# UncertainLab/Enlsip.jl

Measured on NVIDIA B200. Metric: batched CNLS solves/s (n=6,m=128), higher is better.
Workload: dtype f64

## Files before the change

### enlsip.jl_b200/csrc/enl_base.h

```cpp
#pragma once
#include <math.h>
#include <stdint.h>
#include <type_traits>

#if defined(__CUDACC__)
#define ENL_FN __device__
#define ENL_INL __device__ __forceinline__
#define ENL_NOINL __device__ __noinline__
#else
#define ENL_FN
#define ENL_INL inline
#define ENL_NOINL
#endif

namespace enl {

#if defined(__CUDA_ARCH__)
ENL_INL double mul_rn(double a, double b) { return __dmul_rn(a, b); }
ENL_INL double add_rn(double a, double b) { return __dadd_rn(a, b); }
ENL_INL double sub_rn(double a, double b) { return __dsub_rn(a, b); }
ENL_INL double fma_rn(double a, double b, double c) { return fma(a, b, c); }
ENL_INL double div_rn(double a, double b) { return __ddiv_rn(a, b); }
ENL_INL double sqrt_rn(double a) { return __dsqrt_rn(a); }
#else
ENL_INL double mul_rn(double a, double b) { return a * b; }
ENL_INL double add_rn(double a, double b) { return a + b; }
ENL_INL double sub_rn(double a, double b) { return a - b; }
ENL_INL double fma_rn(double a, double b, double c) { return __builtin_fma(a, b, c); }
ENL_INL double div_rn(double a, double b) { return a / b; }
ENL_INL double sqrt_rn(double a) { return sqrt(a); }
#endif

ENL_INL double div_z(double a, double b) { return (a == 0.0) ? a : div_rn(a, b); }

ENL_INL double pow2i(int k) {
    long long b = (long long)(k + 1023) << 52;
#if defined(__CUDA_ARCH__)
    return __longlong_as_double(b);
#else
    double d;
    __builtin_memcpy(&d, &b, 8);
    return d;
#endif
}

#if defined(ENL_COMPACT_CODE) && defined(__CUDA_ARCH__)
#define ENL_DET_EXP_ATTR ENL_NOINL
#else
#define ENL_DET_EXP_ATTR ENL_INL
#endif
ENL_DET_EXP_ATTR double det_exp(double x) {
    const double LOG2E = 1.44269504088896338700e+00;
    const double LN2_HI = 6.93147180369123816490e-01;
    const double LN2_LO = 1.90821492927058770002e-10;
    double xc = fmin(fmax(x, -800.0), 710.0);
    double kd = rint(mul_rn(xc, LOG2E));
    int k = (int)kd;
    double r = fma_rn(-kd, LN2_HI, xc);
    r = fma_rn(-kd, LN2_LO, r);
    double acc = 1.0 / 6227020800.0;
    acc = fma_rn(acc, r, 1.0 / 479001600.0);
    acc = fma_rn(acc, r, 1.0 / 39916800.0);
    acc = fma_rn(acc, r, 1.0 / 3628800.0);
    acc = fma_rn(acc, r, 1.0 / 362880.0);
    acc = fma_rn(acc, r, 1.0 / 40320.0);
    acc = fma_rn(acc, r, 1.0 / 5040.0);
    acc = fma_rn(acc, r, 1.0 / 720.0);
    acc = fma_rn(acc, r, 1.0 / 120.0);
    acc = fma_rn(acc, r, 1.0 / 24.0);
    acc = fma_rn(acc, r, 1.0 / 6.0);
    acc = fma_rn(acc, r, 0.5);
    acc = fma_rn(acc, r, 1.0);
    acc = fma_rn(acc, r, 1.0);
    int k1 = k >> 1;
    int k2 = k - k1;
    double res = mul_rn(mul_rn(acc, pow2i(k1)), pow2i(k2));
    if (x < -745.2) res = 0.0;
    if (x > 709.782712893384) res = INFINITY;
    return (x != x) ? x : res;
}

ENL_INL double det_tanh(double z) {
    double e = det_exp(mul_rn(2.0, z));
    return sub_rn(1.0, div_rn(2.0, add_rn(e, 1.0)));
}

#if defined(__CUDACC__)
template <int G_>
struct DevGroup {
    static constexpr int G = G_;
    unsigned mask;
    int lane;
    __device__ DevGroup() {
        int wl = threadIdx.x & 31;
        lane = wl & (G - 1);
        mask = (G == 32) ? 0xffffffffu : (((1u << G) - 1u) << (wl & ~(G - 1)));
    }
    __device__ __forceinline__ void sync() const {
        if (G > 1) __syncwarp(mask);
    }
    __device__ __forceinline__ double sum(double v) const {
#pragma unroll
        for (int o = G / 2; o > 0; o >>= 1) v += __shfl_xor_sync(mask, v, o, G);
        return v;
    }
    __device__ __forceinline__ double maxv(double v) const {
#pragma unroll
        for (int o = G / 2; o > 0; o >>= 1) v = fmax(v, __shfl_xor_sync(mask, v, o, G));
        return v;
    }
};
#endif

struct HostGroup {
    static constexpr int G = 1;
    int lane = 0;
    void sync() const {}
    double sum(double v) const { return v; }
    double maxv(double v) const { return v; }
};

#if defined(__CUDACC__)
extern __shared__ __align__(16) double enl_smem[];
using vref = int;
ENL_INL vref make_vref(double* p) { return (int)(p - enl_smem); }
ENL_INL vref make_vref(int* p) { return (int)(p - reinterpret_cast<int*>(enl_smem)); }
ENL_INL double& vderef_d(vref o) { return enl_smem[o]; }
ENL_INL int& vderef_i(vref o) { return reinterpret_cast<int*>(enl_smem)[o]; }
#else
using vref = void*;
ENL_INL vref make_vref(double* p) { return p; }
ENL_INL vref make_vref(int* p) { return p; }
#endif

template <int S>
struct SV {
#if defined(__CUDACC__)
    int p;
    ENL_INL double& operator[](int i) const { return enl_smem[p + i * S]; }
#else
    double* p;
    ENL_INL double& operator[](int i) const { return p[i * S]; }
#endif
    ENL_INL SV off(int k) const { return SV{p + k * S}; }
};
template <int S>
struct SI {
#if defined(__CUDACC__)
    int p;
    ENL_INL int& operator[](int i) const { return reinterpret_cast<int*>(enl_smem)[p + i * S]; }
#else
    int* p;
    ENL_INL int& operator[](int i) const { return p[i * S]; }
#endif
};

template <int G, int MS, int NT>
struct DM {
#if defined(__CUDACC__)
    int grp;
    ENL_INL static int lane() { return (int)(threadIdx.x & (G - 1)); }
    ENL_INL static int row_of(int s) { return s * G + lane(); }
    ENL_INL double& at(int s, int c) const { return enl_smem[grp + lane() + (c * MS + s) * NT]; }
    ENL_INL double& row(int r, int c) const { return enl_smem[grp + (c * MS + r / G) * NT + (r % G)]; }
#else
    double* grp;
    ENL_INL static int row_of(int s) { return s * G; }
    ENL_INL double& at(int s, int c) const { return grp[(c * MS + s) * NT]; }
    ENL_INL double& row(int r, int c) const { return grp[(c * MS + r / G) * NT + (r % G)]; }
#endif
    ENL_INL DM cols(int c0) const { return DM{grp + c0 * MS * NT}; }
};

ENL_INL double sq(double v) { return v * v; }
ENL_INL int imin(int a, int b) { return a < b ? a : b; }
ENL_INL int imax(int a, int b) { return a > b ? a : b; }
ENL_INL double sign_of(double a, double b) { return b >= 0.0 ? fabs(a) : -fabs(a); }

ENL_INL double lapy2(double x, double y) {
    double xa = fabs(x), ya = fabs(y);
    double w = fmax(xa, ya), z = fmin(xa, ya);
    if (z == 0.0 || w > 1.7e308) return w;
    return w * sqrt(1.0 + (z / w) * (z / w));
}

constexpr double EPS = 2.220446049250313e-16;
constexpr double SQRT_EPS = 1.4901161193847656e-08;
constexpr double TOL3Z = 1.0536712127723509e-08;

constexpr int EXIT_WOULD_THROW = -99;
constexpr int EXIT_WOULD_HANG = -98;
constexpr int EXIT_CAPACITY = -97;

}
```

### enlsip.jl_b200/csrc/enl_linalg.h

```cpp
#pragma once
#include "enl_base.h"

namespace enl {

#if defined(ENL_HOST_BUILD)
typedef void (*host_dgeqp3_fn)(const int*, const int*, double*, const int*, int*, double*, double*, const int*, int*);
inline host_dgeqp3_fn& host_dgeqp3() { static host_dgeqp3_fn fn = nullptr; return fn; }
inline void host_lapack_qrcp(double* a, int ld, int rows, int cols, double* tau, int* jpvt) {
    static thread_local double work[8192];
    for (int j = 0; j < cols; ++j) jpvt[j] = 0;
    int info = 0;
    const int lwork = 8192;
    host_dgeqp3()(&rows, &cols, a, &ld, jpvt, tau, work, &lwork, &info);
    for (int j = 0; j < cols; ++j) jpvt[j] -= 1;
}
#endif

template <class V>
ENL_NOINL double nrm2_small(V a, int n) {
    double s = 0.0;
#pragma unroll 1
    for (int i = 0; i < n; ++i) s += a[i] * a[i];
    return sqrt(s);
}

template <class V, class VI>
ENL_NOINL void qrcp_small(V a, int ld, int rows, int cols, V tau, VI jpvt, V vn1, V vn2) {
#if defined(ENL_HOST_BUILD)
    if (host_dgeqp3() && rows > 0 && cols > 0) { host_lapack_qrcp(&a[0], ld, rows, cols, &tau[0], &jpvt[0]); return; }
#endif
#pragma unroll 1
    for (int j = 0; j < cols; ++j) {
        jpvt[j] = j;
        double nj = nrm2_small(a.off(j * ld), rows);
        vn1[j] = nj;
        vn2[j] = nj;
    }
    int k = imin(rows, cols);
#pragma unroll 1
    for (int i = 0; i < k; ++i) {
        int pvt = i;
        double best = vn1[i];
#pragma unroll 1
        for (int j = i + 1; j < cols; ++j)
            if (vn1[j] > best) { best = vn1[j]; pvt = j; }
        if (pvt != i) {
#pragma unroll 1
            for (int r = 0; r < rows; ++r) {
                double tmp = a[pvt * ld + r];
                a[pvt * ld + r] = a[i * ld + r];
                a[i * ld + r] = tmp;
            }
            int it = jpvt[pvt]; jpvt[pvt] = jpvt[i]; jpvt[i] = it;
            vn1[pvt] = vn1[i];
            vn2[pvt] = vn2[i];
        }
        double tau_i = 0.0;
        if (i < rows - 1) {
            double alpha = a[i * ld + i];
            double xn = nrm2_small(a.off(i * ld + i + 1), rows - i - 1);
            if (xn != 0.0) {
                double beta = -sign_of(lapy2(alpha, xn), alpha);
                tau_i = (beta - alpha) / beta;
                double sc = 1.0 / (alpha - beta);
#pragma unroll 1
                for (int r = i + 1; r < rows; ++r) a[i * ld + r] *= sc;
                a[i * ld + i] = beta;
            }
        }
        tau[i] = tau_i;
        if (i < cols - 1 && tau_i != 0.0) {
#pragma unroll 1
            for (int c = i + 1; c < cols; ++c) {
                double wv = a[c * ld + i];
#pragma unroll 1
                for (int r = i + 1; r < rows; ++r) wv += a[i * ld + r] * a[c * ld + r];
                wv *= tau_i;
                a[c * ld + i] -= wv;
#pragma unroll 1
                for (int r = i + 1; r < rows; ++r) a[c * ld + r] -= wv * a[i * ld + r];
            }
        }
#pragma unroll 1
        for (int j = i + 1; j < cols; ++j) {
            double v1 = vn1[j];
            if (v1 != 0.0) {
                double tq = fabs(a[j * ld + i]) / v1;
                double temp = fmax(1.0 - tq * tq, 0.0);
                double rq = v1 / vn2[j];
                double temp2 = temp * (rq * rq);
                if (temp2 <= TOL3Z) {
                    if (i < rows - 1) {
                        double nj = nrm2_small(a.off(j * ld + i + 1), rows - i - 1);
                        vn1[j] = nj;
                        vn2[j] = nj;
                    } else {
                        vn1[j] = 0.0;
                        vn2[j] = 0.0;
                    }
                } else {
                    vn1[j] = v1 * sqrt(temp);
                }
            }
        }
    }
}

template <class V>
ENL_NOINL void apply_qt_small(V a, int ld, int rows, int k, V tau, V v) {
#pragma unroll 1
    for (int i = 0; i < k; ++i) {
        double ti = tau[i];
        if (ti == 0.0) continue;
        double wv = v[i];
#pragma unroll 1
        for (int r = i + 1; r < rows; ++r) wv += a[i * ld + r] * v[r];
        wv *= ti;
        v[i] -= wv;
#pragma unroll 1
        for (int r = i + 1; r < rows; ++r) v[r] -= wv * a[i * ld + r];
    }
}

template <class V>
ENL_NOINL void apply_q_small(V a, int ld, int rows, int k, V tau, V v) {
#pragma unroll 1
    for (int i = k - 1; i >= 0; --i) {
        double ti = tau[i];
        if (ti == 0.0) continue;
        double wv = v[i];
#pragma unroll 1
        for (int r = i + 1; r < rows; ++r) wv += a[i * ld + r] * v[r];
        wv *= ti;
        v[i] -= wv;
#pragma unroll 1
        for (int r = i + 1; r < rows; ++r) v[r] -= wv * a[i * ld + r];
    }
}

template <class V, class V2>
ENL_NOINL bool solve_upper_small(V R, int ld, int k, V2 x) {
#pragma unroll 1
    for (int i = k - 1; i >= 0; --i) {
        double s = x[i];
#pragma unroll 1
        for (int j = i + 1; j < k; ++j) s -= R[j * ld + i] * x[j];
        double d = R[i * ld + i];
        if (d == 0.0) return false;
        x[i] = s / d;
    }
    return true;
}

template <class V, class V2>
ENL_NOINL bool solve_upperT_small(V R, int ld, int k, V2 x) {
#pragma unroll 1
    for (int i = 0; i < k; ++i) {
        double s = x[i];
#pragma unroll 1
        for (int j = 0; j < i; ++j) s -= R[i * ld + j] * x[j];
        double d = R[i * ld + i];
        if (d == 0.0) return false;
        x[i] = s / d;
    }
    return true;
}

template <class V>
ENL_NOINL int pseudo_rank(V R, int ld, int len, double eps_rank) {
    if (len <= 0 || fabs(R[0]) < eps_rank) return 0;
    double tol = fabs(R[0]) * sqrt((double)len) * eps_rank;
    int r = 1;
#pragma unroll 1
    while (r < len && fabs(R[(r - 1) * ld + (r - 1)]) > tol) ++r;
    return r - ((r == len && fabs(R[(r - 1) * ld + (r - 1)]) > tol) ? 0 : 1);
}

template <class Grp, int G, int MS, int NT>
struct Dist {
    Grp g;

    ENL_NOINL double colsq(DM<G, MS, NT> a, int c, int r0) const {
        double s = 0.0;
#pragma unroll
        for (int sl = 0; sl < MS; ++sl) {
            int row = sl * G + g.lane;
            double v = a.at(sl, c);
            if (row >= r0) s += v * v;
        }
        return g.sum(s);
    }

    template <class V>
    ENL_NOINL void mul_q_right(DM<G, MS, NT> J, int n, V fa, int ld, int k, V tau) const {
#pragma unroll 1
        for (int i = 0; i < k; ++i) {
            double ti = tau[i];
            if (ti == 0.0) continue;
#pragma unroll
            for (int sl = 0; sl < MS; ++sl) {
                double wv = J.at(sl, i);
#pragma unroll 1
                for (int c = i + 1; c < n; ++c) wv += J.at(sl, c) * fa[i * ld + c];
                wv *= ti;
                J.at(sl, i) -= wv;
#pragma unroll 1
                for (int c = i + 1; c < n; ++c) J.at(sl, c) -= wv * fa[i * ld + c];
            }
        }
    }

    template <class V, class VI>
    ENL_NOINL void qrcp(DM<G, MS, NT> a, int M, int ncols, V tau2, VI jpvt, V vn1, V vn2, V Rout, int ldr) const {
#if defined(ENL_HOST_BUILD)
        if (host_dgeqp3() && G == 1 && NT == 1 && M > 0 && ncols > 0) {
            host_lapack_qrcp(&a.at(0, 0), MS, M, ncols, &tau2[0], &jpvt[0]);
            const int kk = imin(M, ncols);
            for (int c = 0; c < ncols; ++c)
                for (int r = 0; r < kk; ++r) Rout[c * ldr + r] = (r <= c) ? a.row(r, c) : 0.0;
            return;
        }
#endif
#pragma unroll 1
        for (int j = 0; j < ncols; ++j) {
            jpvt[j] = j;
            double nj = sqrt(colsq(a, j, 0));
            vn1[j] = nj;
            vn2[j] = nj;
        }
        int k = imin(M, ncols);
#pragma unroll 1
        for (int i = 0; i < k; ++i) {
            int pvt = i;
            double best = vn1[i];
#pragma unroll 1
            for (int j = i + 1; j < ncols; ++j)
                if (vn1[j] > best) { best = vn1[j]; pvt = j; }
            if (pvt != i) {
#pragma unroll
                for (int sl = 0; sl < MS; ++sl) {
                    double tmp = a.at(sl, pvt);
                    a.at(sl, pvt) = a.at(sl, i);
                    a.at(sl, i) = tmp;
                }
                int it = jpvt[pvt]; jpvt[pvt] = jpvt[i]; jpvt[i] = it;
                vn1[pvt] = vn1[i];
                vn2[pvt] = vn2[i];
            }
            g.sync();
            double tau_i = 0.0;
            if (i < M - 1) {
                double alpha = a.row(i, i);
                double xn = sqrt(colsq(a, i, i + 1));
                if (xn != 0.0) {
                    double beta = -sign_of(lapy2(alpha, xn), alpha);
                    tau_i = (beta - alpha) / beta;
                    double sc = 1.0 / (alpha - beta);
                    g.sync();
#pragma unroll
                    for (int sl = 0; sl < MS; ++sl) {
                        int row = sl * G + g.lane;
                        if (row > i) a.at(sl, i) *= sc;
                        else if (row == i) a.at(sl, i) = beta;
                    }
                }
            }
            tau2[i] = tau_i;
            if (i < ncols - 1 && tau_i != 0.0) {
#pragma unroll 1
                for (int c = i + 1; c < ncols; ++c) {
                    double part = 0.0;
#pragma unroll
                    for (int sl = 0; sl < MS; ++sl) {
                        int row = sl * G + g.lane;
                        double vv = (row > i) ? a.at(sl, i) : ((row == i) ? 1.0 : 0.0);
                        part += vv * a.at(sl, c);
                    }
                    double wv = g.sum(part) * tau_i;
#pragma unroll
                    for (int sl = 0; sl < MS; ++sl) {
                        int row = sl * G + g.lane;
                        if (row > i) a.at(sl, c) -= wv * a.at(sl, i);
                        else if (row == i) a.at(sl, c) -= wv;
                    }
                }
            }
            g.sync();
#pragma unroll 1
            for (int j = i + 1; j < ncols; ++j) {
                double v1 = vn1[j];
                if (v1 != 0.0) {
                    double tq = fabs(a.row(i, j)) / v1;
                    double temp = fmax(1.0 - tq * tq, 0.0);
                    double rq = v1 / vn2[j];
                    double temp2 = temp * (rq * rq);
                    if (temp2 <= TOL3Z) {
                        if (i < M - 1) {
                            double nj = sqrt(colsq(a, j, i + 1));
                            vn1[j] = nj;
                            vn2[j] = nj;
                        } else {
                            vn1[j] = 0.0;
                            vn2[j] = 0.0;
                        }
                    } else {
                        vn1[j] = v1 * sqrt(temp);
                    }
                }
            }
        }
        g.sync();
#pragma unroll 1
        for (int c = 0; c < ncols; ++c)
#pragma unroll 1
            for (int r = 0; r < k; ++r) Rout[c * ldr + r] = (r <= c) ? a.row(r, c) : 0.0;
    }

    template <class V>
    ENL_NOINL void apply_qt(DM<G, MS, NT> a, int k, V tau2, DM<G, MS, NT> d) const {
#pragma unroll 1
        for (int i = 0; i < k; ++i) {
            double ti = tau2[i];
            if (ti == 0.0) continue;
            double part = 0.0;
#pragma unroll
            for (int sl = 0; sl < MS; ++sl) {
                int row = sl * G + g.lane;
                double vv = (row > i) ? a.at(sl, i) : ((row == i) ? 1.0 : 0.0);
                part += vv * d.at(sl, 0);
            }
            double wv = g.sum(part) * ti;
#pragma unroll
            for (int sl = 0; sl < MS; ++sl) {
                int row = sl * G + g.lane;
                if (row > i) d.at(sl, 0) -= wv * a.at(sl, i);
                else if (row == i) d.at(sl, 0) -= wv;
            }
        }
        g.sync();
    }

    template <class V>
    ENL_NOINL void apply_q_regs(DM<G, MS, NT> a, int k, V tau2, double* v) const {
#pragma unroll 1
        for (int i = k - 1; i >= 0; --i) {
            double ti = tau2[i];
            if (ti == 0.0) continue;
            double part = 0.0;
#pragma unroll
            for (int sl = 0; sl < MS; ++sl) {
                int row = sl * G + g.lane;
                double vv = (row > i) ? a.at(sl, i) : ((row == i) ? 1.0 : 0.0);
                part += vv * v[sl];
            }
            double wv = g.sum(part) * ti;
#pragma unroll
            for (int sl = 0; sl < MS; ++sl) {
                int row = sl * G + g.lane;
                double vv = (row > i) ? a.at(sl, i) : ((row == i) ? 1.0 : 0.0);
                v[sl] -= wv * vv;
            }
        }
    }

    ENL_NOINL double prefix_sq(DM<G, MS, NT> d, int len) const {
        double s = 0.0;
#pragma unroll
        for (int sl = 0; sl < MS; ++sl) {
            int row = sl * G + g.lane;
            double v = d.at(sl, 0);
            if (row < len) s += v * v;
        }
        return g.sum(s);
    }
};

}
```

### enlsip.jl_b200/csrc/enl_solver.h

```cpp
#pragma once
#include "enl_base.h"
#include "enl_linalg.h"
#include "enl_families.h"

namespace enl {

struct Options {
    int max_iter;
    int scaling;
    int jac_mode;
    int second_derivatives;
    double time_limit;
    double eps_abs;
    double eps_rel;
    double eps_x;
    double eps_c;
    double eps_rank;
};

constexpr int MAX_N = 32;
struct Bounds {
    int nlo, nup;
    int lo_idx[MAX_N], up_idx[MAX_N];
    double lo_val[MAX_N], up_val[MAX_N];
};

constexpr int TRACE_HDR = 16;

template <class Fam, int G, int NT>
struct Layout {
    static constexpr int N = Fam::N, M = Fam::M, Q = Fam::Q, NNL = Fam::Q + Fam::NI;
    static constexpr int LMAX = NNL + Fam::MAXB;
    static constexpr int T = (LMAX < N) ? LMAX : N;
    static constexpr int PPC = NT / G;
    static constexpr int MS = (M + G - 1) / G;
    static constexpr int NS = (N > LMAX) ? N : LMAX;
    enum : int {
        oX = 0, oXPREV = oX + N, oXNEW = oXPREV + N, oCX = oXNEW + N, oCNEW = oCX + LMAX, oA = oCNEW + LMAX,
        oGRADF = oA + LMAX * N, oW = oGRADF + N, oWNEW = oW + LMAX, oK = oWNEW + LMAX, oACX = oK + 4 * LMAX,
        oAA = oACX + T, oDSC = oAA + T * N, oFA = oDSC + T, oTAUA = oFA + N * T, oFL = oTAUA + T,
        oTAUL = oFL + T * T, oR2 = oTAUL + T, oTAU2 = oR2 + N * N, oLAM = oTAU2 + N, oB = oLAM + T, oP = oB + T,
        oY = oP + N, oAP = oY + N, oAAP = oAP + LMAX, oV1C = oAAP + T, oVN1 = oV1C + LMAX, oVN2 = oVN1 + N,
        oS1 = oVN2 + N, oS2 = oS1 + NS, oS3 = oS2 + NS, oS4 = oS3 + NS, oS5 = oS4 + NS, oNW = oS5 + NS,
        oFS = oNW + 3 * N * N, nD = oFS + Fam::NSCAL
    };
    enum : int { iACT = 0, iINACT = iACT + LMAX, iPERMA = iINACT + LMAX, iPERML = iPERMA + T, iPERM2 = iPERML + T,
                 iPOS = iPERM2 + N, nI = iPOS + T };
    static constexpr int DCOLS = N + 2 + Fam::NDCOLS;
    static constexpr size_t smem_bytes() {
        return (size_t)nD * PPC * 8 + (size_t)DCOLS * MS * NT * 8 + (size_t)nI * PPC * 4;
    }
};

struct IterRec {
    int t, rankA, rankJ2, dimA, dimJ2, code, index_del, index_alpha_upp, nb_newton;
    bool restart, add, del;
    double alpha, beta, progress, predicted_reduction, grad_res, speed;
};

struct Outputs {
    double* x;
    double* f;
    int* exit_code;
    int* status;
    int* iters;
    int* nact;
    int* active;
    int* counters;
    double* trace;
    int trace_cap;
};

template <class Fam, class Grp, int NT>
struct Solver {
    static constexpr int G = Grp::G;
    using LY = Layout<Fam, G, NT>;
    static constexpr int N = LY::N, M = LY::M, Q = LY::Q, NNL = LY::NNL, LMAX = LY::LMAX, T = LY::T, PPC = LY::PPC,
                         MS = LY::MS;
    using V = SV<PPC>;
    using VI = SI<PPC>;
    using D = DM<G, MS, NT>;

    V x, xprev, xnew, cx, cnew, A, gradf, w, wnew, K, acx, aA, dsc, FA, tauA, FL, tauL, R2, tau2, lam, b, p, y, Ap, aAp,
        v1c, vn1, vn2, s1, s2, s3, s4, s5, nw;
    VI active, inactive, permA, permL, perm2, posidx;
    D dR, dJ, dF, dD, dY;
    V fs;
    using FCtx = typename Fam::template Ctx<D, V>;
    ENL_INL Grp grp() const { return Grp(); }
    ENL_INL Dist<Grp, G, MS, NT> dst() const { return Dist<Grp, G, MS, NT>(); }
    ENL_INL FCtx fctx() const { return FCtx{dY, fs}; }
    const Options& opt;
    const Bounds& bnd;

    int l, t, k_iter, ndetail, exit_code;
    int n_res, n_cons, n_jres, n_jcons;
    bool threw, hang;
    bool j2_factored;
    IterRec cur, prev;
    double rx_sum, active_cx_sum, f_detail, rdot_x1, cdot_x1, rdot_prev, cdot_prev;
    double jp_r, jp_jp;
    double t_start;

    ENL_FN Solver(double* small, int* ints, double* distbase, int pid, const Options& o, const Bounds& bb)
        : opt(o), bnd(bb) {
#if defined(__CUDACC__)
        int s = (int)(small - enl_smem) + pid;
#else
        double* s = small + pid;
#endif
        auto mk = [&](int off) { return V{s + off * PPC}; };
        x = mk(LY::oX); xprev = mk(LY::oXPREV); xnew = mk(LY::oXNEW); cx = mk(LY::oCX); cnew = mk(LY::oCNEW);
        A = mk(LY::oA); gradf = mk(LY::oGRADF); w = mk(LY::oW); wnew = mk(LY::oWNEW); K = mk(LY::oK);
        acx = mk(LY::oACX); aA = mk(LY::oAA); dsc = mk(LY::oDSC); FA = mk(LY::oFA); tauA = mk(LY::oTAUA);
        FL = mk(LY::oFL); tauL = mk(LY::oTAUL); R2 = mk(LY::oR2); tau2 = mk(LY::oTAU2); lam = mk(LY::oLAM);
        b = mk(LY::oB); p = mk(LY::oP); y = mk(LY::oY); Ap = mk(LY::oAP); aAp = mk(LY::oAAP); v1c = mk(LY::oV1C);
        vn1 = mk(LY::oVN1); vn2 = mk(LY::oVN2); s1 = mk(LY::oS1); s2 = mk(LY::oS2); s3 = mk(LY::oS3);
        s4 = mk(LY::oS4); s5 = mk(LY::oS5); nw = mk(LY::oNW); fs = mk(LY::oFS);
#if defined(__CUDACC__)
        int ii = (int)(ints - reinterpret_cast<int*>(enl_smem)) + pid;
#else
        int* ii = ints + pid;
#endif
        auto mi = [&](int off) { return VI{ii + off * PPC}; };
        active = mi(LY::iACT); inactive = mi(LY::iINACT); permA = mi(LY::iPERMA); permL = mi(LY::iPERML);
        perm2 = mi(LY::iPERM2); posidx = mi(LY::iPOS);
#if defined(__CUDACC__)
        int grpb = (int)(distbase - enl_smem) + pid * G;
#else
        double* grpb = distbase + pid * G;
#endif
        D all{grpb};
        dR = all; dJ = all.cols(1); dF = dJ; dD = all.cols(1 + N); dY = all.cols(2 + N);
        l = NNL + bnd.nlo + bnd.nup;
    }

    ENL_FN void load_x(V src, double* xv) const {
#pragma unroll
        for (int j = 0; j < N; ++j) xv[j] = src[j];
    }

    ENL_NOINL void eval_point(const double* xv, double* rn, V cout) {
        Fam::template residuals<Grp, MS>(fctx(), grp(), xv, rn);
        double cnl[NNL > 0 ? NNL : 1];
        if (NNL > 0) Fam::template constraints<MS>(fctx(), xv, cnl);
#pragma unroll 1
        for (int i = 0; i < NNL; ++i) cout[i] = cnl[i];
#pragma unroll 1
        for (int j = 0; j < bnd.nlo; ++j) cout[NNL + j] = sub_rn(xv[bnd.lo_idx[j]], bnd.lo_val[j]);
#pragma unroll 1
        for (int j = 0; j < bnd.nup; ++j) cout[NNL + bnd.nlo + j] = sub_rn(bnd.up_val[j], xv[bnd.up_idx[j]]);
    }

    ENL_FN double sumsq_regs(const double* rn) const {
        double s = 0.0;
#pragma unroll
        for (int sl = 0; sl < MS; ++sl) s += rn[sl] * rn[sl];
        return grp().sum(s);
    }

    const double* mat_J = nullptr;
    ENL_NOINL void eval_res_jacobian() {
        if (mat_J) {
#pragma unroll
            for (int sl = 0; sl < MS; ++sl) {
                const int row = sl * G + grp().lane;
#pragma unroll
                for (int j = 0; j < N; ++j) dJ.at(sl, j) = (row < M) ? mat_J[(size_t)j * M + row] : 0.0;
            }
            j2_factored = false;
            grp().sync();
            return;
        }
        double xv[N];
        load_x(x, xv);
        double out[MS * N];
        if (opt.jac_mode == 0) {
            Fam::template jac_residuals<Grp, MS>(fctx(), grp(), xv, out);
        } else {
            double r0[MS], dl[N];
#pragma unroll
            for (int sl = 0; sl < MS; ++sl) r0[sl] = dR.at(sl, 0);
#pragma unroll
            for (int j = 0; j < N; ++j) dl[j] = mul_rn(fmax(fabs(xv[j]), 1.0), SQRT_EPS);
            fd_res(xv, r0, dl, out);
        }
#pragma unroll
        for (int sl = 0; sl < MS; ++sl)
#pragma unroll
            for (int j = 0; j < N; ++j) dJ.at(sl, j) = out[sl * N + j];
        j2_factored = false;
        grp().sync();
    }

    template <class F2 = Fam>
    ENL_FN typename std::enable_if<F2::HAS_FAST_FD>::type fd_res(const double* xv, const double* r0, const double* dl,
                                                                 double* out) {
        F2::template fd_jac_residuals<Grp, MS>(fctx(), grp(), xv, r0, dl, out);
    }
    template <class F2 = Fam>
    ENL_FN typename std::enable_if<!F2::HAS_FAST_FD>::type fd_res(const double* xv, const double* r0, const double* dl,
                                                                  double* out) {
        double xf[N], rf[MS];
#pragma unroll
        for (int j = 0; j < N; ++j) {
#pragma unroll
            for (int i = 0; i < N; ++i) xf[i] = xv[i];
            xf[j] = add_rn(xv[j], dl[j]);
            F2::template residuals<Grp, MS>(fctx(), grp(), xf, rf);
#pragma unroll
            for (int sl = 0; sl < MS; ++sl) out[sl * N + j] = div_z(sub_rn(rf[sl], r0[sl]), dl[j]);
        }
    }

    ENL_NOINL void eval_cons_jacobian() {
        double xv[N];
        load_x(x, xv);
        if (NNL > 0) {
            double An[(NNL > 0 ? NNL : 1) * N];
            if (opt.jac_mode == 0) {
                Fam::template jac_constraints<MS>(fctx(), xv, An);
            } else {
                double xf[N], cf[NNL > 0 ? NNL : 1];
#pragma unroll 1
                for (int j = 0; j < N; ++j) {
                    double dj = mul_rn(fmax(fabs(xv[j]), 1.0), SQRT_EPS);
#pragma unroll 1
                    for (int i = 0; i < N; ++i) xf[i] = xv[i];
                    xf[j] = add_rn(xv[j], dj);
                    Fam::template constraints<MS>(fctx(), xf, cf);
#pragma unroll 1
                    for (int i = 0; i < NNL; ++i) An[i * N + j] = div_z(sub_rn(cf[i], cx[i]), dj);
                }
            }
#pragma unroll 1
            for (int i = 0; i < NNL * N; ++i) A[i] = An[i];
        }
    }

    ENL_NOINL void init_bound_rows() {
#pragma unroll 1
        for (int j = 0; j < bnd.nlo; ++j)
#pragma unroll 1
// ... 103 lines not shown
                dsc[i] = 1.0 / row;
            }
        }
    }

    ENL_NOINL void factor_A() {
#pragma unroll 1
        for (int c = 0; c < t; ++c)
#pragma unroll 1
            for (int r = 0; r < N; ++r) FA[c * N + r] = aA[c * N + r];
        qrcp_small(FA, N, N, t, tauA, permA, vn1, vn2);
    }
    ENL_NOINL void factor_L11() {
#pragma unroll 1
        for (int c = 0; c < t; ++c)
#pragma unroll 1
            for (int r = 0; r < t; ++r) FL[c * T + r] = (c <= r) ? FA[r * N + c] : 0.0;
        qrcp_small(FL, T, t, t, tauL, permL, vn1, vn2);
    }

    ENL_NOINL void first_lagrange() {
        int pr = pseudo_rank(FA, N, t, opt.eps_rank);
#pragma unroll 1
        for (int i = 0; i < N; ++i) s1[i] = gradf[i];
        apply_qt_small(FA, N, N, t, tauA, s1);
#pragma unroll 1
        for (int i = 0; i < t; ++i) s2[i] = (i < pr) ? s1[i] : 0.0;
        if (!solve_upper_small(FA, N, pr, s2)) threw = true;
        double gr = 0.0;
#pragma unroll 1
        for (int i = pr; i < N; ++i) gr += s1[i] * s1[i];
        cur.grad_res = (N > pr) ? sqrt(gr) : 0.0;
#pragma unroll 1
        for (int j = 0; j < t; ++j) s3[j] = (j < pr) ? -acx[permA[j]] : 0.0;
        if (!solve_upperT_small(FA, N, pr, s3)) threw = true;
        if (!solve_upper_small(FA, N, pr, s3)) threw = true;
#pragma unroll 1
        for (int j = 0; j < t; ++j) lam[permA[j]] = s2[j] + s3[j];
        if (opt.scaling)
#pragma unroll 1
            for (int i = 0; i < t; ++i) lam[i] = lam[i] * dsc[i];
    }

    ENL_NOINL void second_lagrange() {
        int pr = pseudo_rank(FA, N, t, SQRT_EPS);
        double v[MS];
        {
            const int kq = imin(M, N - cur.rankA);
#pragma unroll
            for (int sl = 0; sl < MS; ++sl) {
                int row = sl * G + grp().lane;
                v[sl] = (row >= kq) ? -dD.at(sl, 0) : 0.0;
            }
            dst().apply_q_regs(dF, kq, tau2, v);
        }
#pragma unroll 1
        for (int j = 0; j < t; ++j) {
            double s = 0.0;
#pragma unroll
            for (int sl = 0; sl < MS; ++sl) s += dJ.at(sl, j) * v[sl];
            s1[j] = grp().sum(s);
        }
#pragma unroll 1
        for (int j = pr; j < t; ++j) s1[j] = 0.0;
        if (!solve_upper_small(FA, N, pr, s1)) threw = true;
#pragma unroll 1
        for (int j = 0; j < t; ++j) lam[permA[j]] = s1[j];
        if (opt.scaling)
#pragma unroll 1
            for (int i = 0; i < t; ++i) lam[i] = lam[i] * dsc[i];
    }

    ENL_NOINL int check_constraint_deletion(double grad_res) {
        double lam_max = 1.0;
        if (t > 0) {
            lam_max = 0.0;
#pragma unroll 1
            for (int i = 0; i < t; ++i) lam_max = fmax(lam_max, fabs(lam[i]));
        }
        double sq_rel = SQRT_EPS * lam_max;
        int s = 0;
        if (t > Q) {
            double e = sq_rel;
#pragma unroll 1
            for (int i = Q + 1; i <= t; ++i) {
                double row_i = opt.scaling ? 1.0 / dsc[i - 1] : dsc[i - 1];
                double v = row_i * lam[i - 1];
                if (v <= sq_rel && v <= e) { e = v; s = i; }
            }
            if (grad_res > -e * 10.0) s = 0;
        }
        return s;
    }

    ENL_FN void minmax_lagrangian_mult(double& sigmin, double& lam_abs_max) {
        lam_abs_max = 0.0;
        sigmin = INFINITY;
        if (t > Q) {
#pragma unroll 1
            for (int i = 0; i < t; ++i) lam_abs_max = fmax(lam_abs_max, fabs(lam[i]));
#pragma unroll 1
            for (int i = Q; i < t; ++i) {
                double rows = opt.scaling ? 1.0 / dsc[i] : dsc[i];
                double li = lam[i];
                if (li * rows <= -SQRT_EPS && li < sigmin) sigmin = li;
            }
        }
    }

    ENL_NOINL void sub_search_direction(int rankA, int dimA, int dimJ2, int code) {
        const int k2 = N - rankA;
        const int kq = imin(M, k2);
        if (code == 1) {
#pragma unroll 1
            for (int j = 0; j < t; ++j) { double v = -acx[permA[j]]; b[j] = v; y[j] = v; }
            if (!solve_upperT_small(FA, N, t, y)) threw = true;
        } else {
#pragma unroll 1
            for (int j = 0; j < t; ++j) s1[j] = -acx[permA[j]];
            apply_qt_small(FL, T, t, t, tauL, s1);
#pragma unroll 1
            for (int j = 0; j < t; ++j) b[j] = s1[j];
            if (dimA > t || dimA < 0) { threw = true; dimA = imax(0, imin(dimA, t)); }
#pragma unroll 1
            for (int j = 0; j < t; ++j) s2[j] = (j < dimA) ? s1[j] : 0.0;
            if (!solve_upper_small(FL, T, dimA, s2)) threw = true;
#pragma unroll 1
            for (int j = 0; j < t; ++j) s3[permL[j]] = s2[j];
#pragma unroll 1
            for (int j = 0; j < rankA; ++j) y[j] = s3[j];
        }
#pragma unroll
        for (int sl = 0; sl < MS; ++sl) {
            double acc = 0.0;
#pragma unroll 1
            for (int c = 0; c < rankA; ++c) acc += dJ.at(sl, c) * y[c];
            dD.at(sl, 0) = -acc - dR.at(sl, 0);
        }
        grp().sync();
        dst().apply_qt(dF, kq, tau2, dD);
        if (dimJ2 > kq || dimJ2 < 0) { threw = true; dimJ2 = imax(0, imin(dimJ2, kq)); }
#pragma unroll 1
        for (int j = 0; j < dimJ2; ++j) s2[j] = dD.row(j, 0);
        if (!solve_upper_small(R2, N, dimJ2, s2)) threw = true;
#pragma unroll 1
        for (int j = 0; j < k2; ++j) y[rankA + perm2[j]] = (j < dimJ2) ? s2[j] : 0.0;
#pragma unroll 1
        for (int j = 0; j < N; ++j) p[j] = y[j];
        apply_q_small(FA, N, N, t, tauA, p);
    }

    ENL_NOINL void gn_search_direction(int rankA) {
        int code = (rankA == t) ? 1 : -1;
        dst().mul_q_right(dJ, N, FA, N, t, tauA);
        const int k2 = N - rankA;
        dF = dJ.cols(rankA);
        grp().sync();
        dst().qrcp(dF, M, k2, tau2, perm2, vn1, vn2, R2, N);
        j2_factored = true;
        int rankJ2 = pseudo_rank(R2, N, imin(M, k2), opt.eps_rank);
        sub_search_direction(rankA, rankA, rankJ2, code);
        cur.rankA = rankA;
        cur.rankJ2 = rankJ2;
        cur.dimA = rankA;
        cur.dimJ2 = rankJ2;
    }

    ENL_NOINL void update_working_set() {
        factor_A();
        first_lagrange();
        int s = check_constraint_deletion(cur.grad_res);
        if (s != 0) {
            cur.index_del = 0;
            cur.del = false;
            if (opt.scaling) {
#pragma unroll 1
                for (int i = 0; i < t; ++i) {
                    int id = active[i] - 1;
#pragma unroll 1
                    for (int c = 0; c < N; ++c) aA[i * N + c] = A[id * N + c] * dsc[i];
                }
                factor_A();
            }
        }
#pragma unroll 1
        for (int pass = 0; pass < 2; ++pass) {
            int rankA = pseudo_rank(FA, N, t, opt.eps_rank);
            factor_L11();
            gn_search_direction(rankA);
            if (pass == 0 && t == rankA && cur.rankJ2 == imin(M, N - rankA)) {
                second_lagrange();
                int s2 = check_constraint_deletion(0.0);
                if (s2 != 0) {
                    int id = active[s2 - 1];
#pragma unroll 1
                    for (int i = s2; i <= t - 1; ++i) {
                        lam[i - 1] = lam[i];
                        dsc[i - 1] = dsc[i];
                        acx[i - 1] = acx[i];
#pragma unroll 1
                        for (int c = 0; c < N; ++c) aA[(i - 1) * N + c] = aA[i * N + c];
                    }
                    ws_remove(s2);
                    cur.del = true;
                    cur.index_del = id;
                    eval_res_jacobian();
                    factor_A();
                    continue;
                }
            }
            break;
        }
    }

    ENL_FN int gn_previous_step(V tau, double tau_prk, int mindim, V rho, double rho_prk, int prank) {
        const double tau_max = 2e-1, rho_min = 5e-1;
        int pm1 = prank - 1;
        if (mindim > pm1) return mindim;
        int kk = pm1;
#pragma unroll 1
        while ((tau[kk - 1] >= tau_max * tau_prk || rho[kk - 1] <= rho_min * rho_prk) && kk > mindim) --kk;
        return (kk > mindim) ? kk : imax(mindim, pm1);
    }

    ENL_NOINL int subspace_min_previous_step(V tau, V rho, int len, double rho_prk, double c1, int pseudo_rk, int pdim,
                                          double progress, double plp, double prelin_prev, double prev_alpha) {
        const double stepb = 2e-1, pgb1 = 3e-1, pgb2 = 1e-1, predb = 7e-1, rlenb = 2.0, c2 = 1e2;
        auto ok = [&](int i) { if (i < 1 || i > len) { threw = true; return false; } return true; };
        if (prev_alpha < stepb && progress <= pgb1 * plp * plp && progress <= pgb2 * prelin_prev * prelin_prev) {
            int dim = imax(1, pdim - 1);
            if (pdim > 1) {
                if (!ok(dim)) return pseudo_rk;
                if (rho[dim - 1] > c1 * rho_prk) return dim;
            }
        }
        int dim = pdim;
        bool first_cond = false;
        if (pdim < len) {
            if (!ok(dim) || !ok(dim + 1)) return pseudo_rk;
            first_cond = ((rho[dim - 1] > predb * rho_prk) && (rlenb * tau[dim - 1] < tau[dim])) || (c2 * tau[dim - 1] < tau[dim]);
        }
        if (first_cond) return dim;
        int i1 = pdim - 1;
        if (i1 <= 0) return pseudo_rk;
        int best = 0;
#pragma unroll 1
        for (int i = i1; i <= pdim; ++i) {
            if (!ok(i)) return pseudo_rk;
            if (rho[i - 1] > predb * rho_prk) { if (best == 0) best = i; }
        }
        return best == 0 ? pseudo_rk : best;
    }

    ENL_NOINL int determine_solving_dim(int pdim, int rankR, double plp, double obj_progress, double prelin_prev, V R, int ld,
                                     V yv, double prev_alpha, bool restart) {
        const double c1 = 0.1;
        int newdim = rankR;
        int mindim = 1;
        if (rankR > 0) {
            V sd = s4, rh = s5;
            sd[0] = fabs(yv[0]);
            rh[0] = fabs(yv[0] / R[0]);
#pragma unroll 1
            for (int i = 1; i < rankR; ++i) {
                double a = yv[i], r = yv[i] / R[i * ld + i];
                rh[i] = sqrt(rh[i - 1] * rh[i - 1] + r * r);
                sd[i] = sqrt(sd[i - 1] * sd[i - 1] + a * a);
            }
            double nrm_sd = sd[rankR - 1], nrm_rh = rh[rankR - 1];
            double dsum = 0.0, psimax = 0.0;
#pragma unroll 1
            for (int i = 0; i < rankR; ++i) {
                dsum += sd[i] * sd[i];
                double psi = sqrt(dsum) * fabs(R[i * ld + i]);
                if (psi > psimax) { psimax = psi; mindim = i + 1; }
            }
            if (!restart) {
                int suggested;
                if (pdim == rankR || pdim <= 0)
                    suggested = gn_previous_step(sd, nrm_sd, mindim, rh, nrm_rh, rankR);
                else
                    suggested = subspace_min_previous_step(sd, rh, rankR, nrm_rh, c1, rankR, pdim, obj_progress, plp,
                                                           prelin_prev, prev_alpha);
                newdim = imax(mindim, suggested);
            } else {
                newdim = imax(0, imin(rankR, pdim));
            }
        }
        return newdim;
    }

    ENL_NOINL void choose_subspace_dimensions(int rankA, int rankJ2, bool restart, int& dimA, int& dimJ2) {
        const double alpha_low = 0.2;
        double prev_alpha = prev.alpha;
        int pdA;
        const int k2 = N - rankA;
        const int kq = imin(M, k2);
        if (rankA <= 0) {
            dimA = 0;
            pdA = 0;
#pragma unroll
            for (int sl = 0; sl < MS; ++sl) dD.at(sl, 0) = -dR.at(sl, 0);
        } else {
            pdA = abs(prev.dimA) + t - prev.t;
            if (pdA > t) { threw = true; pdA = t; }
            double sb = 0.0, sa = 0.0;
#pragma unroll 1
            for (int j = 0; j < t; ++j) {
                sb += b[j] * b[j];
                if (j < pdA) sa += b[j] * b[j];
            }
            double nrm_b = sqrt(sb), nrm_b_asprev = sqrt(sa);
            double cprog = cdot_prev - active_cx_sum;
            dimA = determine_solving_dim(pdA, rankA, nrm_b, cprog, nrm_b_asprev, FL, T, b, prev_alpha, restart);
            if (dimA > t || rankA - dimA < 0) { threw = true; dimA = imin(dimA, rankA); }
#pragma unroll 1
            for (int j = 0; j < rankA; ++j) s2[j] = (j < dimA) ? b[j] : 0.0;
            if (!solve_upper_small(FL, T, dimA, s2)) threw = true;
#pragma unroll 1
            for (int i = 0; i < rankA; ++i) {
                double acc = 0.0;
#pragma unroll 1
                for (int j = 0; j < rankA; ++j)
                    if (permL[j] == i) acc += s2[j];
                s3[i] = acc;
            }
#pragma unroll
            for (int sl = 0; sl < MS; ++sl) {
                double acc = 0.0;
#pragma unroll 1
                for (int c = 0; c < rankA; ++c) acc += dJ.at(sl, c) * s3[c];
                dD.at(sl, 0) = -(dR.at(sl, 0) + acc);
            }
        }
        grp().sync();
        if (rankJ2 > 0) dst().apply_qt(dF, kq, tau2, dD);
        int pdJ = abs(prev.dimJ2) + prev.t - t;
        if (pdJ > M) { threw = true; pdJ = M; }
        double nrm_d_asprev = sqrt(dst().prefix_sq(dD, pdJ));
        double nrm_d = sqrt(dst().prefix_sq(dD, M));
        double rprog = rdot_prev - rx_sum;
        if (rankJ2 > M) { threw = true; }
#pragma unroll 1
        for (int j = 0; j < rankJ2 && j < M; ++j) s2[j] = dD.row(j, 0);
        dimJ2 = determine_solving_dim(pdJ, rankJ2, nrm_d, rprog, nrm_d_asprev, R2, N, s2, prev_alpha, restart);
        if (!restart && prev_alpha >= alpha_low) {
            dimA = imax(dimA, pdA);
            dimJ2 = imax(dimJ2, pdJ);
        }
    }

    ENL_NOINL int check_gn_direction(double b1nrm, double d1nrm, double d1nrm_as_km1, double dnrm, double active_c_sum,
                                  int rankA, bool restart, bool added, bool deleted, double& beta_k) {
        const double delta = 1e-1;
        const double c1 = 0.5, c2 = 0.1, c3 = 4.0, c4 = 10.0, c5 = 0.05;
        beta_k = sqrt(d1nrm * d1nrm + b1nrm * b1nrm);
        int method = 1;
        bool newton_or_restart = (prev.code == 2) || restart;
        bool first_iter = (k_iter == 0);
        bool submin_prev = prev.code == -1;
        bool add_or_del = added || deleted;
        bool conv_lower = beta_k < c1 * prev.beta;
        bool progress_not_close = (prev.progress > c2 * prev.predicted_reduction) && (dnrm <= c3 * beta_k);
        if (newton_or_restart || (!first_iter && (submin_prev || !(add_or_del || conv_lower || progress_not_close)))) {
            method = -1;
            double nonlin_k = sqrt(d1nrm * d1nrm + active_c_sum);
            double nonlin_km1 = sqrt(d1nrm_as_km1 * d1nrm_as_km1 + active_c_sum);
            bool to_reduce = false;
            if (Q < t) {
                bool any_ge = false, any_neg = false;
#pragma unroll 1
                for (int i = Q; i < t; ++i) {
                    double rows = opt.scaling ? 1.0 / dsc[i] : dsc[i];
                    if (lam[i] * rows >= -SQRT_EPS) any_ge = true;
                    if (lam[i] < 0) any_neg = true;
                }
                to_reduce = to_reduce || (any_ge && any_neg);
            }
            if (l - t > 0) {
                bool any_small = false;
#pragma unroll 1
                for (int j = 0; j < l - t; ++j)
                    if (cx[inactive[j] - 1] < delta) any_small = true;
                to_reduce = to_reduce || any_small;
            }
            bool newton_previously = (prev.code == 2) && !deleted;
            bool cond4 = active_c_sum > c2;
            bool cond5 = deleted || added || to_reduce || (t == N && t == rankA);
            double eps_ = fmax(1e-2, 10.0 * EPS);
            bool cond6 = !((l == Q) || (rankA <= t)) && !((beta_k < eps_ * dnrm) || (b1nrm < eps_ && M == N - t));
            if (newton_previously || !(cond4 || cond5 || cond6)) {
                bool cond7 = (prev.alpha < c5 && nonlin_km1 < c2 * nonlin_k) || (M == N - t);
                bool cond8 = !(dnrm <= c4 * beta_k);
                if (newton_previously || cond7 || cond8) method = 2;
            }
        }
        return method;
    }

    ENL_NOINL bool newton_search_direction(int rankA) {
        const double e1 = 6.055454452393343e-06;
        V Gm = nw, Em = nw.off(N * N), Wm = nw.off(2 * N * N);
        if (t == rankA) {
#pragma unroll 1
            for (int j = 0; j < t; ++j) y[j] = -acx[permA[j]];
            if (!solve_upperT_small(FA, N, t, y)) threw = true;
        } else {
#pragma unroll 1
            for (int j = 0; j < t; ++j) s1[j] = -acx[permA[j]];
            apply_qt_small(FL, T, t, t, tauL, s1);
#pragma unroll 1
            for (int j = 0; j < rankA; ++j) s2[j] = s1[j];
            if (!solve_upper_small(FL, T, rankA, s2)) threw = true;
#pragma unroll 1
            for (int i = 0; i < rankA; ++i) {
                double acc = 0.0;
#pragma unroll 1
                for (int j = 0; j < rankA; ++j)
                    if (permL[j] == i) acc += s2[j];
                y[i] = acc;
            }
        }
        if (rankA == N) { threw = true; return true; }
        eval_res_jacobian();
        dst().mul_q_right(dJ, N, FA, N, t, tauA);
        grp().sync();
        double xv[N], xw[N], fa[MS], fb[MS];
        load_x(x, xv);
        double rr[MS];
#pragma unroll
        for (int sl = 0; sl < MS; ++sl) rr[sl] = dR.at(sl, 0);
#pragma unroll 1
        for (int kk = 0; kk < N; ++kk)
#pragma unroll 1
            for (int j = 0; j <= kk; ++j) {
                double ek = fmax(fabs(xv[kk]), 1.0) * e1;
                double ej = fmax(fabs(xv[j]), 1.0) * e1;
                double cacc[LMAX];
#pragma unroll 1
                for (int q4 = 0; q4 < 4; ++q4) {
#pragma unroll 1
                    for (int i = 0; i < N; ++i) xw[i] = xv[i];
                    double sj = (q4 == 0 || q4 == 2) ? ej : -ej;
                    double sk = (q4 < 2) ? ek : -ek;
                    xw[j] = add_rn(xw[j], sj);
                    xw[kk] = add_rn(xw[kk], sk);
                    eval_point(xw, fb, cnew);
                    n_res += 1; n_cons += 1;
                    double sgn = (q4 == 0 || q4 == 3) ? 1.0 : -1.0;
                    if (q4 == 0) {
#pragma unroll
                        for (int sl = 0; sl < MS; ++sl) fa[sl] = fb[sl];
#pragma unroll 1
                        for (int i = 0; i < l; ++i) cacc[i] = cnew[i];
                    } else {
#pragma unroll
                        for (int sl = 0; sl < MS; ++sl) fa[sl] = fa[sl] + sgn * fb[sl];
#pragma unroll 1
                        for (int i = 0; i < l; ++i) cacc[i] = cacc[i] + sgn * cnew[i];
                    }
                }
                double sr = 0.0;
#pragma unroll
                for (int sl = 0; sl < MS; ++sl) sr += fa[sl] * rr[sl];
                sr = grp().sum(sr) / (4 * ej * ek);
                double sc = 0.0;
#pragma unroll 1
                for (int i = 0; i < t; ++i) sc += cacc[active[i] - 1] * lam[i];
                sc = sc / (4.0 * ek * ej);
                Gm[j * N + kk] = sr - sc;
                Gm[kk * N + j] = sr - sc;
            }
#pragma unroll 1
        for (int c = 0; c < N; ++c) apply_qt_small(FA, N, N, t, tauA, Gm.off(c * N));
#pragma unroll 1
        for (int r = 0; r < N; ++r) {
#pragma unroll 1
            for (int c = 0; c < N; ++c) s1[c] = Gm[c * N + r];
            apply_qt_small(FA, N, N, t, tauA, s1);
#pragma unroll 1
            for (int c = 0; c < N; ++c) Em[c * N + r] = s1[c];
        }
        if (t > rankA) {
            if (t != N) { threw = true; return true; }
#pragma unroll 1
            for (int c = 0; c < N; ++c)
#pragma unroll 1
                for (int r = 0; r < N; ++r) Gm[c * N + r] = Em[permL[c] * N + permL[r]];
#pragma unroll 1
            for (int i = 0; i < N * N; ++i) Em[i] = Gm[i];
        }
        const int k2 = N - rankA;
#pragma unroll 1
        for (int a = 0; a < k2; ++a) {
#pragma unroll 1
            for (int c = 0; c < N; ++c) {
                double s = 0.0;
#pragma unroll
                for (int sl = 0; sl < MS; ++sl) s += dJ.at(sl, rankA + a) * dJ.at(sl, c);
                s1[c] = grp().sum(s);
            }
            double sjr = 0.0;
#pragma unroll
            for (int sl = 0; sl < MS; ++sl) sjr += dJ.at(sl, rankA + a) * rr[sl];
            sjr = grp().sum(sjr);
            double dacc = 0.0;
#pragma unroll 1
            for (int c = 0; c < rankA; ++c) dacc += (Em[c * N + (rankA + a)] + s1[c]) * y[c];
            s2[a] = -dacc - sjr;
#pragma unroll 1
            for (int c2 = 0; c2 < k2; ++c2) Wm[c2 * N + a] = Em[(rankA + c2) * N + (rankA + a)] + s1[rankA + c2];
        }
#pragma unroll 1
        for (int a = 0; a < k2; ++a)
#pragma unroll 1
            for (int c = a; c < k2; ++c) {
                double v = (Wm[c * N + a] + Wm[a * N + c]) * 0.5;
                Gm[c * N + a] = v;
            }
#pragma unroll 1
        for (int j = 0; j < k2; ++j) {
            double ajj = Gm[j * N + j];
#pragma unroll 1
            for (int i = 0; i < j; ++i) ajj -= Gm[j * N + i] * Gm[j * N + i];
            if (!(ajj > 0.0)) {
#pragma unroll 1
                for (int i = 0; i < N; ++i) p[i] = 0.0;
#pragma unroll 1
                for (int i = 0; i < N; ++i) y[i] = 0.0;
                return true;
            }
            ajj = sqrt(ajj);
            Gm[j * N + j] = ajj;
#pragma unroll 1
            for (int c = j + 1; c < k2; ++c) {
                double v = Gm[c * N + j];
#pragma unroll 1
                for (int i = 0; i < j; ++i) v -= Gm[j * N + i] * Gm[c * N + i];
                Gm[c * N + j] = v / ajj;
            }
        }
        solve_upperT_small(Gm, N, k2, s2);
        solve_upper_small(Gm, N, k2, s2);
#pragma unroll 1
        for (int a = 0; a < k2; ++a) y[rankA + a] = s2[a];
#pragma unroll 1
        for (int j = 0; j < N; ++j) p[j] = y[j];
        apply_q_small(FA, N, N, t, tauA, p);
        return false;
    }

    ENL_NOINL int search_direction_analys() {
        const int rankA = cur.rankA, rankJ2 = cur.rankJ2;
        double sb = 0.0;
#pragma unroll 1
        for (int j = 0; j < cur.dimA; ++j) sb += b[j] * b[j];
        double nrm_b1_gn = sqrt(sb);
        double nrm_d_gn = sqrt(dst().prefix_sq(dD, M));
        double nrm_d1_gn = sqrt(dst().prefix_sq(dD, cur.dimJ2));
        int pd = prev.dimJ2 + prev.t - t - 1;
        if (pd > M) { threw = true; pd = M; }
        double nrm_d1_asprev = sqrt(dst().prefix_sq(dD, pd));
        bool restart = cur.restart;
        int error_code = 0;
        double beta;
        int method = check_gn_direction(nrm_b1_gn, nrm_d1_gn, nrm_d1_asprev, nrm_d_gn, active_cx_sum, rankA, restart,
                                        cur.add, cur.del, beta);
        int dimA = rankA, dimJ2 = rankJ2;
        if (method == -1) {
#pragma unroll 1
            for (int j = 0; j < t; ++j) s1[j] = -acx[permA[j]];
            apply_qt_small(FL, T, t, t, tauL, s1);
#pragma unroll 1
            for (int j = 0; j < t; ++j) b[j] = s1[j];
            choose_subspace_dimensions(rankA, rankJ2, restart, dimA, dimJ2);
            if (!threw) sub_search_direction(rankA, dimA, dimJ2, -1);
            if (dimA == rankA && dimJ2 == rankJ2) method = 1;
        } else if (method == 2) {
// ... 898 lines not shown
```

Before: 2.024 million.

## Register-block Householder updates in mul_q_right, qrcp and apply_qt

Makes N a compile-time parameter of the distributed linear-algebra helper. mul_q_right now loads row chunks of J into registers and applies all reflectors there before writing back. qrcp updates several trailing columns per pass, combining their warp reductions into one batched shuffle and optionally holding the column values in registers. apply_qt keeps the right-hand side in registers across reflectors. The aim is fewer shared-memory round trips and shuffle rounds, at the cost of more register pressure and FMA contraction that may change rounding.

New measurement: 2.016 million (median of 6 runs). No clear change (-0.4%).

```diff
diff --git a/enlsip.jl_b200/csrc/enl_base.h b/enlsip.jl_b200/csrc/enl_base.h
--- a/enlsip.jl_b200/csrc/enl_base.h
+++ b/enlsip.jl_b200/csrc/enl_base.h
@@ -30,6 +30,14 @@
 ENL_INL double div_rn(double a, double b) { return a / b; }
 ENL_INL double sqrt_rn(double a) { return sqrt(a); }
 #endif
+
+ENL_INL double mad_c(double a, double b, double c) {
+#if defined(__CUDA_ARCH__)
+    return fma(a, b, c);
+#else
+    return a * b + c;
+#endif
+}
 
 ENL_INL double div_z(double a, double b) { return (a == 0.0) ? a : div_rn(a, b); }
 
@@ -104,6 +112,13 @@
         for (int o = G / 2; o > 0; o >>= 1) v += __shfl_xor_sync(mask, v, o, G);
         return v;
     }
+    template <int W>
+    __device__ __forceinline__ void sum_n(double (&v)[W]) const {
+#pragma unroll
+        for (int o = G / 2; o > 0; o >>= 1)
+#pragma unroll
+            for (int j = 0; j < W; ++j) v[j] += __shfl_xor_sync(mask, v[j], o, G);
+    }
     __device__ __forceinline__ double maxv(double v) const {
 #pragma unroll
         for (int o = G / 2; o > 0; o >>= 1) v = fmax(v, __shfl_xor_sync(mask, v, o, G));
@@ -117,6 +132,8 @@
     int lane = 0;
     void sync() const {}
     double sum(double v) const { return v; }
+    template <int W>
+    void sum_n(double (&)[W]) const {}
     double maxv(double v) const { return v; }
 };
 
diff --git a/enlsip.jl_b200/csrc/enl_linalg.h b/enlsip.jl_b200/csrc/enl_linalg.h
--- a/enlsip.jl_b200/csrc/enl_linalg.h
+++ b/enlsip.jl_b200/csrc/enl_linalg.h
@@ -176,11 +176,23 @@
     return r - ((r == len && fabs(R[(r - 1) * ld + (r - 1)]) > tol) ? 0 : 1);
 }
 
-template <class Grp, int G, int MS, int NT>
+template <class Grp, int G, int MS, int NT, int N>
 struct Dist {
     Grp g;
-
-    ENL_NOINL double colsq(DM<G, MS, NT> a, int c, int r0) const {
+    using D = DM<G, MS, NT>;
+
+    static constexpr int NCHUNK = (N + 7) / 8;
+    static constexpr int CW = (N + NCHUNK - 1) / NCHUNK;
+    static constexpr bool HOLD = CW * MS <= 32;
+    static constexpr int rows_per_chunk() {
+        int r = (32 / N < 1) ? 1 : 32 / N;
+        r = (r > MS) ? MS : r;
+        while (MS % r) --r;
+        return r;
+    }
+    static constexpr int RS = rows_per_chunk();
+
+    ENL_NOINL double colsq(D a, int c, int r0) const {
         double s = 0.0;
 #pragma unroll
         for (int sl = 0; sl < MS; ++sl) {
@@ -192,26 +204,43 @@
     }
 
     template <class V>
-    ENL_NOINL void mul_q_right(DM<G, MS, NT> J, int n, V fa, int ld, int k, V tau) const {
-#pragma unroll 1
-        for (int i = 0; i < k; ++i) {
-            double ti = tau[i];
-            if (ti == 0.0) continue;
-#pragma unroll
-            for (int sl = 0; sl < MS; ++sl) {
-                double wv = J.at(sl, i);
-#pragma unroll 1
-                for (int c = i + 1; c < n; ++c) wv += J.at(sl, c) * fa[i * ld + c];
-                wv *= ti;
-                J.at(sl, i) -= wv;
-#pragma unroll 1
-                for (int c = i + 1; c < n; ++c) J.at(sl, c) -= wv * fa[i * ld + c];
-            }
+    ENL_NOINL void mul_q_right(D J, V fa, int ld, int k, V tau) const {
+        if (k <= 0) return;
+#pragma unroll 1
+        for (int s0 = 0; s0 < MS; s0 += RS) {
+            double x[RS][N];
+#pragma unroll
+            for (int r = 0; r < RS; ++r)
+#pragma unroll
+                for (int c = 0; c < N; ++c) x[r][c] = J.at(s0 + r, c);
+#pragma unroll
+            for (int i = 0; i < N; ++i) {
+                const double ti = (i < k) ? tau[i] : 0.0;
+                if (ti != 0.0) {
+                    double f[N];
+#pragma unroll
+                    for (int c = i + 1; c < N; ++c) f[c] = fa[i * ld + c];
+#pragma unroll
+                    for (int r = 0; r < RS; ++r) {
+                        double wv = x[r][i];
+#pragma unroll
+                        for (int c = i + 1; c < N; ++c) wv = mad_c(x[r][c], f[c], wv);
+                        wv *= ti;
+                        x[r][i] -= wv;
+#pragma unroll
+                        for (int c = i + 1; c < N; ++c) x[r][c] = mad_c(-wv, f[c], x[r][c]);
+                    }
+                }
+            }
+#pragma unroll
+            for (int r = 0; r < RS; ++r)
+#pragma unroll
+                for (int c = 0; c < N; ++c) J.at(s0 + r, c) = x[r][c];
         }
     }
 
     template <class V, class VI>
-    ENL_NOINL void qrcp(DM<G, MS, NT> a, int M, int ncols, V tau2, VI jpvt, V vn1, V vn2, V Rout, int ldr) const {
+    ENL_NOINL void qrcp(D a, int M, int ncols, V tau2, VI jpvt, V vn1, V vn2, V Rout, int ldr) const {
 #if defined(ENL_HOST_BUILD)
         if (host_dgeqp3() && G == 1 && NT == 1 && M > 0 && ncols > 0) {
             host_lapack_qrcp(&a.at(0, 0), MS, M, ncols, &tau2[0], &jpvt[0]);
@@ -268,20 +297,37 @@
             tau2[i] = tau_i;
             if (i < ncols - 1 && tau_i != 0.0) {
 #pragma unroll 1
-                for (int c = i + 1; c < ncols; ++c) {
-                    double part = 0.0;
+                for (int c0 = i + 1; c0 < ncols; c0 += CW) {
+                    double part[CW];
+                    double x[HOLD ? CW : 1][HOLD ? MS : 1];
+#pragma unroll
+                    for (int j = 0; j < CW; ++j) part[j] = 0.0;
 #pragma unroll
                     for (int sl = 0; sl < MS; ++sl) {
                         int row = sl * G + g.lane;
-                        double vv = (row > i) ? a.at(sl, i) : ((row == i) ? 1.0 : 0.0);
-                        part += vv * a.at(sl, c);
-                    }
-                    double wv = g.sum(part) * tau_i;
+                        double ai = a.at(sl, i);
+                        double vv = (row > i) ? ai : ((row == i) ? 1.0 : 0.0);
+#pragma unroll
+                        for (int j = 0; j < CW; ++j) {
+                            double ac = a.at(sl, imin(c0 + j, ncols - 1));
+                            if (HOLD) x[HOLD ? j : 0][HOLD ? sl : 0] = ac;
+                            part[j] = mad_c(vv, ac, part[j]);
+                        }
+                    }
+                    g.sum_n(part);
+                    double wv[CW];
+#pragma unroll
+                    for (int j = 0; j < CW; ++j) wv[j] = part[j] * tau_i;
 #pragma unroll
                     for (int sl = 0; sl < MS; ++sl) {
                         int row = sl * G + g.lane;
-                        if (row > i) a.at(sl, c) -= wv * a.at(sl, i);
-                        else if (row == i) a.at(sl, c) -= wv;
+                        double ai = a.at(sl, i);
+#pragma unroll
+                        for (int j = 0; j < CW; ++j) {
+                            double ac = HOLD ? x[HOLD ? j : 0][HOLD ? sl : 0] : a.at(sl, imin(c0 + j, ncols - 1));
+                            double nv = (row > i) ? mad_c(-wv[j], ai, ac) : ac - wv[j];
+                            if (row >= i && c0 + j < ncols) a.at(sl, c0 + j) = nv;
+                        }
                     }
                 }
             }
@@ -317,7 +363,10 @@
     }
 
     template <class V>
-    ENL_NOINL void apply_qt(DM<G, MS, NT> a, int k, V tau2, DM<G, MS, NT> d) const {
+    ENL_NOINL void apply_qt(D a, int k, V tau2, D d) const {
+        double dv[MS];
+#pragma unroll
+        for (int sl = 0; sl < MS; ++sl) dv[sl] = d.at(sl, 0);
 #pragma unroll 1
         for (int i = 0; i < k; ++i) {
             double ti = tau2[i];
@@ -327,21 +376,23 @@
             for (int sl = 0; sl < MS; ++sl) {
                 int row = sl * G + g.lane;
                 double vv = (row > i) ? a.at(sl, i) : ((row == i) ? 1.0 : 0.0);
-                part += vv * d.at(sl, 0);
+                part = mad_c(vv, dv[sl], part);
             }
             double wv = g.sum(part) * ti;
 #pragma unroll
             for (int sl = 0; sl < MS; ++sl) {
                 int row = sl * G + g.lane;
-                if (row > i) d.at(sl, 0) -= wv * a.at(sl, i);
-                else if (row == i) d.at(sl, 0) -= wv;
-            }
-        }
+                if (row > i) dv[sl] = mad_c(-wv, a.at(sl, i), dv[sl]);
+                else if (row == i) dv[sl] -= wv;
+            }
+        }
+#pragma unroll
+        for (int sl = 0; sl < MS; ++sl) d.at(sl, 0) = dv[sl];
         g.sync();
     }
 
     template <class V>
-    ENL_NOINL void apply_q_regs(DM<G, MS, NT> a, int k, V tau2, double* v) const {
+    ENL_NOINL void apply_q_regs(D a, int k, V tau2, double* v) const {
 #pragma unroll 1
         for (int i = k - 1; i >= 0; --i) {
             double ti = tau2[i];
@@ -363,7 +414,7 @@
         }
     }
 
-    ENL_NOINL double prefix_sq(DM<G, MS, NT> d, int len) const {
+    ENL_NOINL double prefix_sq(D d, int len) const {
         double s = 0.0;
 #pragma unroll
         for (int sl = 0; sl < MS; ++sl) {
diff --git a/enlsip.jl_b200/csrc/enl_solver.h b/enlsip.jl_b200/csrc/enl_solver.h
--- a/enlsip.jl_b200/csrc/enl_solver.h
+++ b/enlsip.jl_b200/csrc/enl_solver.h
@@ -88,7 +88,7 @@
     V fs;
     using FCtx = typename Fam::template Ctx<D, V>;
     ENL_INL Grp grp() const { return Grp(); }
-    ENL_INL Dist<Grp, G, MS, NT> dst() const { return Dist<Grp, G, MS, NT>(); }
+    ENL_INL Dist<Grp, G, MS, NT, N> dst() const { return Dist<Grp, G, MS, NT, N>(); }
     ENL_INL FCtx fctx() const { return FCtx{dY, fs}; }
     const Options& opt;
     const Bounds& bnd;
@@ -498,7 +498,7 @@
 
     ENL_NOINL void gn_search_direction(int rankA) {
         int code = (rankA == t) ? 1 : -1;
-        dst().mul_q_right(dJ, N, FA, N, t, tauA);
+        dst().mul_q_right(dJ, FA, N, t, tauA);
         const int k2 = N - rankA;
         dF = dJ.cols(rankA);
         grp().sync();
@@ -769,7 +769,7 @@
         }
         if (rankA == N) { threw = true; return true; }
         eval_res_jacobian();
-        dst().mul_q_right(dJ, N, FA, N, t, tauA);
+        dst().mul_q_right(dJ, FA, N, t, tauA);
         grp().sync();
         double xv[N], xw[N], fa[MS], fb[MS];
         load_x(x, xv);
```
